# netneurolab/pypyls

Hardware: AMD Instinct MI355X
Metric: resamples/sec (perm+boot), behavioral_pls X(500x200000)/Y(500x50) fp64 (higher is better)
Workload: dtype f64

## Files before the change

pypyls_amd/csrc/plsx_k_prep.h:

```cpp
#pragma once
#include "plsx_common.h"


static __global__ void k_colmean(const double* __restrict__ X, int S, int B, double* __restrict__ mean)
{
    int b = blockIdx.x * blockDim.x + threadIdx.x;
    if (b >= B) return;
    double s = 0.0;
    for (int i = 0; i < S; ++i) s += X[(size_t)i * B + b];
    mean[b] = s / (double)S;
}

static __global__ void k_center_pad(const double* __restrict__ X, const double* __restrict__ mean,
                             int S, int B, double* __restrict__ Xc, int ldx)
{
    int b = blockIdx.x * blockDim.x + threadIdx.x;
    int i = blockIdx.y;
    if (b >= B || i >= S) return;
    Xc[(size_t)i * ldx + b] = X[(size_t)i * B + b] - mean[b];
}

static __global__ void k_cell_scale(const double* __restrict__ Xc, int ldx, int B, int J,
                             const int* __restrict__ cell_start, const int* __restrict__ cell_len,
                             double* __restrict__ Xn)
// ... 32 lines not shown
    const int* row_local = nullptr;
    const int* slice_cell0 = nullptr;
};

static __global__ void k_build_A_behav(const double* __restrict__ Y0, long long y_stride, int T, int S,
                                const int* __restrict__ cell_start, const int* __restrict__ cell_len,
                                const int* __restrict__ xsrc, const int* __restrict__ ysrc,
                                GroupLayout lay, int covariance, int scaled,
                                double* __restrict__ Afrag, size_t group_stride,
                                double* __restrict__ mom_n, int nmom_pad, int dense_ld = 0,
                                double* __restrict__ Amom = nullptr, size_t mom_stride = 0,
                                const int* __restrict__ rank = nullptr, int mom_pairs = PLSX_MOM_PAIRS,
                                int chain_cap = 0, int mom_row0 = -1, int row0 = 0)
{
    extern __shared__ double sm_b[];
    const int r = blockIdx.x, j = blockIdx.y;
    const int g = r / lay.n, rr = r % lay.n;
    const double* Y = Y0 + (size_t)r * y_stride;
    const int start = cell_start[j], len = cell_len[j];
    const int* xs = xsrc ? xsrc + (size_t)r * S : nullptr;
    const int* ys = ysrc ? ysrc + (size_t)r * S : nullptr;
    double* mean = sm_b;
    double* rstd = sm_b + T;
    __shared__ int s_cnt;
    const int tid = threadIdx.x;

    if (tid == 0) {
        int c = 0;
        for (int p = start; p < start + len; ++p) c += (xs ? xs[p] : p) >= 0;
        s_cnt = c;
    }
    __syncthreads();
    const int cnt = s_cnt;
    for (int t = tid; t < T; t += blockDim.x) {
        double s = 0.0;
        for (int p = start; p < start + len; ++p) {
            int xi = xs ? xs[p] : p;
            if (xi < 0) continue;
            int yi = ys ? ys[p] : p;
            s += Y[(size_t)yi * T + t];
        }
        double m = s / (double)cnt;
        double q = 0.0;
        for (int p = start; p < start + len; ++p) {
            int xi = xs ? xs[p] : p;
            if (xi < 0) continue;
            int yi = ys ? ys[p] : p;
            double d = Y[(size_t)yi * T + t] - m;
            q += d * d;
        }
        mean[t] = m;
        rstd[t] = covariance ? 1.0 : 1.0 / sqrt(q / (double)(cnt - 1));
    }
    __syncthreads();
    double* A = Afrag + (size_t)g * group_stride;
    const double inv_nm1 = 1.0 / (double)(cnt - 1);
    const int total = len * T;
    const bool sliced = lay.gps > 0 && !dense_ld;
    int* nxt = reinterpret_cast<int*>(sm_b + 2 * T);
    int* nfirst = nxt + len;
    const bool unique = !xs || chain_cap < 0;
    const bool chains = !unique && 2 * len <= chain_cap;
    if (chains) {
        for (int pl = tid; pl < len; pl += blockDim.x) nfirst[pl] = 0;
        __syncthreads();
        for (int pl = tid; pl < len; pl += blockDim.x) {
            const int xi = xs[start + pl];
            int nx = -1;
            if (xi >= 0)
                for (int q = pl + 1; q < len; ++q)
                    if (xs[start + q] == xi) { nx = q; break; }
            nxt[pl] = nx;
            if (nx >= 0) nfirst[nx] = 1;
        }
        __syncthreads();
    }
    for (int idx = tid; idx < total; idx += blockDim.x) {
        int pl = idx / T, t = idx - pl * T;
        int p = start + pl;
        int xi = xs ? xs[p] : p;
        if (xi < 0) continue;
        double v;
        if (chains) {
            if (nfirst[pl]) continue;
            v = 0.0;
            for (int q = pl; q >= 0; q = nxt[q]) {
                const int yq = ys ? ys[start + q] : start + q;
                v += (Y[(size_t)yq * T + t] - mean[t]) * rstd[t] * inv_nm1;
            }
        } else {
            int yi = ys ? ys[p] : p;
            v = (Y[(size_t)yi * T + t] - mean[t]) * rstd[t] * inv_nm1;
        }
        int row = rr * lay.Tp + row0 + j * T + t;
        double* dst;
        if (dense_ld) dst = Afrag + ((size_t)r * lay.Tp + j * T + t) * dense_ld + xi;
        else if (sliced) {
            const int grow = j * T + t;
            dst = Afrag + ((size_t)r * lay.gps + lay.row_slice[grow]) * group_stride +
                  afrag_off(lay.row_local[grow], xi, lay.MT);
        } else dst = A + afrag_off(row, rank ? rank[(size_t)r * S + xi] : xi, lay.MT);
        if (chains || unique) *dst = v;
        else atomicAdd(dst, v);
    }
    auto put_weight = [&](double* d0, double* d1, int pl) {
        if (chains) {
            if (nfirst[pl]) return;
            double c = 0.0;
            for (int q = pl; q >= 0; q = nxt[q]) c += 1.0;
            *d0 = c; *d1 = c;
        } else if (unique) { *d0 = 1.0; *d1 = 1.0; }
        else { atomicAdd(d0, 1.0); atomicAdd(d1, 1.0); }
    };
    if (scaled && sliced) {
        const int sa = lay.row_slice[j * T], sb = lay.row_slice[j * T + T - 1];
        for (int sl = sa; sl <= sb; ++sl) {
            const size_t gg = (size_t)r * lay.gps + sl;
            double* As = Afrag + gg * group_stride;
            const int mrow = j - lay.slice_cell0[sl];
            for (int pl = tid; pl < len; pl += blockDim.x) {
                int p = start + pl;
                int xi = xs ? xs[p] : p;
                if (xi < 0) continue;
                put_weight(As + afrag_off(lay.w0 * 16 + mrow, xi, lay.MT), As + afrag_off(lay.sq0 * 16 + mrow, xi, lay.MT), pl);
            }
            if (tid == 0) mom_n[gg * nmom_pad + mrow] = (double)cnt;
        }
    } else if (scaled && Amom) {
        const int pair = r * lay.J + j;
        double* Am = Amom + (size_t)(pair / mom_pairs) * mom_stride;
        const int mrow = pair % mom_pairs, mmt = mom_row0 >= 0 ? mom_pairs / 16 : mom_pairs / 8;
        for (int pl = tid; pl < len; pl += blockDim.x) {
            int p = start + pl;
            int xi = xs ? xs[p] : p;
            if (xi < 0) continue;
            if (mom_row0 >= 0)
                put_weight(A + afrag_off(mom_row0 + j, rank[(size_t)r * S + xi], lay.MT), Am + afrag_off(mrow, xi, mmt), pl);
            else
                put_weight(Am + afrag_off(mrow, xi, mmt), Am + afrag_off(mom_pairs + mrow, xi, mmt), pl);
        }
        if (tid == 0) mom_n[pair] = (double)cnt;
    } else if (scaled) {
        for (int pl = tid; pl < len; pl += blockDim.x) {
            int p = start + pl;
            int xi = xs ? xs[p] : p;
            if (xi < 0) continue;
            int mrow = rr * lay.J + j;
            put_weight(A + afrag_off(lay.w0 * 16 + mrow, xi, lay.MT), A + afrag_off(lay.sq0 * 16 + mrow, xi, lay.MT), pl);
        }
        if (tid == 0) mom_n[(size_t)g * nmom_pad + rr * lay.J + j] = (double)cnt;
    }
}

static __global__ __launch_bounds__(256)
void k_build_A_proj(const double* __restrict__ Y0, long long y_stride, int T, int S,
                    const int* __restrict__ cell_start, const int* __restrict__ cell_len,
                    const int* __restrict__ ysrc, const double* __restrict__ V0, int L,
                    int n, int Tp, int MT, double* __restrict__ Afrag, size_t group_stride)
{
    extern __shared__ double sm_b[];
    const int r = blockIdx.x, j = blockIdx.y;
    const int g = r / n, rr = r % n;
    const double* Y = Y0 + (size_t)r * y_stride;
    const int start = cell_start[j], len = cell_len[j];
    const int* ys = ysrc ? ysrc + (size_t)r * S : nullptr;
    double* mean = sm_b;
    double* rstd = sm_b + T;
    const int tid = threadIdx.x;
    for (int t = tid; t < T; t += blockDim.x) {
        double s = 0.0;
        for (int p = start; p < start + len; ++p) s += Y[(size_t)(ys ? ys[p] : p) * T + t];
        const double m = s / (double)len;
        double q = 0.0;
        for (int p = start; p < start + len; ++p) {
            const double d = Y[(size_t)(ys ? ys[p] : p) * T + t] - m;
            q += d * d;
        }
        mean[t] = m;
        rstd[t] = 1.0 / sqrt(q / (double)(len - 1));
    }
    __syncthreads();
    double* A = Afrag + (size_t)g * group_stride;
    const double inv_nm1 = 1.0 / (double)(len - 1);
    const double* Vj = V0 + (size_t)j * T * L;
    const int total = len * L;
    for (int idx = tid; idx < total; idx += blockDim.x) {
        const int pl = idx / L, l = idx - pl * L;
        const int p = start + pl;
        const double* y = Y + (size_t)(ys ? ys[p] : p) * T;
        double v = 0.0;
        for (int t = 0; t < T; ++t)
            v = __builtin_fma((y[t] - mean[t]) * rstd[t] * inv_nm1, Vj[(size_t)t * L + l], v);
        A[afrag_off(rr * Tp + l, p, MT)] = v;
    }
}

static __global__ void k_build_A_mc(int S, int J, int n_cond, int mean_centering,
                             const int* __restrict__ cell_of_pos,
                             const int* __restrict__ xsrc, GroupLayout lay,
                             double* __restrict__ Afrag, size_t group_stride, int dense_ld = 0, int chain_cap = 0)
{
    extern __shared__ int sm_mc[];
    __shared__ int cnt[PLSX_MAX_CELLS];
    const int r = blockIdx.x;
    const int g = r / lay.n, rr = r % lay.n;
    const int* xs = xsrc ? xsrc + (size_t)r * S : nullptr;
    const int tid = threadIdx.x;
    for (int j = tid; j < J; j += blockDim.x) cnt[j] = 0;
    __syncthreads();
    for (int p = tid; p < S; p += blockDim.x)
        if ((xs ? xs[p] : p) >= 0) atomicAdd(&cnt[cell_of_pos[p]], 1);
    __syncthreads();
    const int n_groups = J / n_cond;
    int ntot = 0;
    for (int j = 0; j < J; ++j) ntot += cnt[j];
    double* A = Afrag + (size_t)g * group_stride;
    int* nxt = sm_mc;
    int* nfirst = sm_mc + S;
    const bool unique = !xs || chain_cap < 0;
    const bool chains = !unique && 2 * S <= chain_cap;
    if (chains) {
        for (int p = tid; p < S; p += blockDim.x) nfirst[p] = 0;
        __syncthreads();
        for (int p = tid; p < S; p += blockDim.x) {
            const int xi = xs[p];
            int nx = -1;
            if (xi >= 0)
                for (int q = p + 1; q < S; ++q)
                    if (xs[q] == xi) { nx = q; break; }
            nxt[p] = nx;
            if (nx >= 0) nfirst[nx] = 1;
        }
        __syncthreads();
    }
    auto coef_of = [&](int p, int j2) -> double {
        const int j = cell_of_pos[p];
        const int gj = j / n_cond, cj = j % n_cond;
        const double own = 1.0 / (double)cnt[j];
        double coef = (j2 == j) ? own : 0.0;
        if (mean_centering == 0) {
            if (j2 / n_cond == gj) {
                int ngrp = 0;
                for (int c = 0; c < n_cond; ++c) ngrp += cnt[gj * n_cond + c];
                coef -= 1.0 / (double)ngrp;
            }
        } else if (mean_centering == 1) {
            if (j2 % n_cond == cj) coef -= own / (double)n_groups;
        } else {
            coef -= 1.0 / (double)ntot;
        }
        return coef;
    };
    for (int p = tid; p < S; p += blockDim.x) {
        int xi = xs ? xs[p] : p;
        if (xi < 0) continue;
        if (chains && nfirst[p]) continue;
        for (int j2 = 0; j2 < J; ++j2) {
            double coef;
            if (chains) {
                coef = 0.0;
                for (int q = p; q >= 0; q = nxt[q]) coef += coef_of(q, j2);
            } else coef = coef_of(p, j2);
            if (coef == 0.0) continue;
            double* dst = dense_ld ? Afrag + ((size_t)r * lay.Tp + j2) * dense_ld + xi
                                   : A + afrag_off(rr * lay.Tp + j2, xi, lay.MT);
            if (chains || unique) *dst = coef;
            else atomicAdd(dst, coef);
        }
    }
}

__device__ __forceinline__ size_t mfrag_index(int t, int l, int nks_t, int LT)
{
    const int chunk = (l >> 4) / PLSX_LT_CHUNK, lt = (l >> 4) - chunk * PLSX_LT_CHUNK;
    const int ltc = min(PLSX_LT_CHUNK, LT - chunk * PLSX_LT_CHUNK);
    return (size_t)chunk * PLSX_LT_CHUNK * nks_t * 64 + ((size_t)(t >> 2) * ltc + lt) * 64 + (t & 3) * 16 + (l & 15);
}

static __global__ __launch_bounds__(256)
void k_build_W(const double* __restrict__ Adense, int ld, int S, int Tp, int L,
               const double* __restrict__ Mfrag, int nks_t, int LT, int npg_w, int MT,
               double* __restrict__ Afrag, size_t group_stride)
{
    extern __shared__ __attribute__((aligned(16))) double sM[];
    const int r = blockIdx.x, tid = threadIdx.x;
    const double* M = Mfrag + (size_t)r * nks_t * LT * 64;
    for (int idx = tid; idx < Tp * L; idx += blockDim.x) {
        const int t = idx / L, l = idx - t * L;
        sM[idx] = M[mfrag_index(t, l, nks_t, LT)];
    }
    __syncthreads();
    const double* A = Adense + (size_t)r * Tp * ld;
    double* out = Afrag + (size_t)(r / npg_w) * group_stride;
    const int row0 = (r % npg_w) * L;
    for (int i = tid; i < S; i += blockDim.x)
        for (int l0 = 0; l0 < L; l0 += 8) {
            double w[8] = {0, 0, 0, 0, 0, 0, 0, 0};
            for (int t = 0; t < Tp; ++t) {
                const double a = A[(size_t)t * ld + i];
#pragma unroll
                for (int u = 0; u < 8; ++u) w[u] += a * sM[t * L + min(l0 + u, L - 1)];
            }
#pragma unroll
            for (int u = 0; u < 8; ++u)
                if (l0 + u < L) out[afrag_off(row0 + l0 + u, i, MT)] = w[u];
        }
}

static __global__ __launch_bounds__(256)
void k_build_Vd(const double* __restrict__ Adense, int ld, int S, int Tp, int L,
                const double* __restrict__ Mfrag, int nks_t, int LT, double* __restrict__ Vd)
{
    extern __shared__ __attribute__((aligned(16))) double sM[];
    const int r = blockIdx.x, tid = threadIdx.x;
    const double* M = Mfrag + (size_t)r * nks_t * LT * 64;
    for (int idx = tid; idx < Tp * L; idx += blockDim.x) {
        const int t = idx / L, l = idx - t * L;
        sM[idx] = M[mfrag_index(t, l, nks_t, LT)];
    }
    __syncthreads();
    const double* A = Adense + (size_t)r * Tp * ld;
    double* out = Vd + (size_t)r * L * S;
    for (int i = tid; i < S; i += blockDim.x)
        for (int l0 = 0; l0 < L; l0 += 8) {
            double w[8] = {0, 0, 0, 0, 0, 0, 0, 0};
            for (int t = 0; t < Tp; ++t) {
                const double a = A[(size_t)t * ld + i];
#pragma unroll
                for (int u = 0; u < 8; ++u) w[u] += a * sM[t * L + min(l0 + u, L - 1)];
            }
#pragma unroll
            for (int u = 0; u < 8; ++u)
                if (l0 + u < L) out[(size_t)(l0 + u) * S + i] = w[u];
        }
}

static __global__ void k_cell_moments(const double* __restrict__ Xc, int ldx, int B, int J,
                               const int* __restrict__ cell_start, const int* __restrict__ cell_len,
                               double* __restrict__ S1, double* __restrict__ S2)
{
    const int b = blockIdx.x * blockDim.x + threadIdx.x;
    if (b >= B) return;
    for (int j = 0; j < J; ++j) {
        const int r0 = cell_start[j], n = cell_len[j];
        double s = 0.0, q = 0.0;
        for (int i = r0; i < r0 + n; ++i) { const double x = Xc[(size_t)i * ldx + b]; s += x; q += x * x; }
// ... 149 lines not shown
```

pypyls_amd/csrc/plsx_k_xprod.h:

```cpp
#pragma once
#include <type_traits>
#include <utility>

template <class F, int... I>
__device__ __forceinline__ void xprod_static_for(F&& f, std::integer_sequence<int, I...>)
{
    (f(std::integral_constant<int, I>()), ...);
}
#include "plsx_common.h"
#include "plsx_k_prep.h"

#define PLSX_RSRC_FLAGS 0x00020000
template <int NT, int PASSES, bool EVEN, int STAGE>
__device__ __forceinline__ void stage_copy_buf(const double* src, double* dst, int tid, int wave)
{
    __amdgpu_buffer_rsrc_t rs = __builtin_amdgcn_make_buffer_rsrc((void*)src, (short)0, 0x7fffffff,
                                                                   PLSX_RSRC_FLAGS);
    const int voff = tid * 16;
#pragma unroll
    for (int p = 0; p < PASSES; ++p) {
        if (EVEN || p * NT + wave * 64 < STAGE / 2) {
            __builtin_amdgcn_raw_ptr_buffer_load_lds(
                rs, (__attribute__((address_space(3))) void*)(dst + (size_t)(p * NT + wave * 64) * 2),
                16, voff, p * NT * 16, 0, 0);
        }
    }
}

__device__ __forceinline__ double load_x_buf(const double* rowbase, int voff)
{
    __amdgpu_buffer_rsrc_t rs = __builtin_amdgcn_make_buffer_rsrc((void*)rowbase, (short)0, 0x7fffffff,
                                                                   PLSX_RSRC_FLAGS);
    return __builtin_bit_cast(double, __builtin_amdgcn_raw_buffer_load_b64(rs, voff, 0, 0));
}

template <int CTRL>
__device__ __forceinline__ double dpp_row_f64(double v)
{
    const int vl = __double2loint(v), vh = __double2hiint(v);
    const int lo = __builtin_amdgcn_update_dpp(vl, vl, CTRL, 0xf, 0xf, false);
    const int hi = __builtin_amdgcn_update_dpp(vh, vh, CTRL, 0xf, 0xf, false);
    return __hiloint2double(hi, lo);
}

#define PLSX_ACC_PITCH 80
template <int MT, int NW, int KT, int NSQ, int EPI = 0>
__global__ __launch_bounds__(NW * 64, 2)
void k_xprod(const double* __restrict__ Afrag, size_t group_stride,
             const double* __restrict__ X, int ldx, int nks,
             double* __restrict__ R, int ldr, int rows_per_group,
             const int* __restrict__ out_row, const int* __restrict__ mom_idx,
             const double* __restrict__ mom_n, int nmom_pad,
             int n_groups, int ncolblk, double* __restrict__ mom_out, SplitEpi se, int ntab)
{
    extern __shared__ __attribute__((aligned(16))) double smem[];
    constexpr int NT = NW * 64;
    constexpr int STAGE = KT * MT * 64;
    constexpr int STAGE_LDS = ((STAGE + 127) / 128) * 128;
    constexpr int PASSES = (STAGE + NT * 2 - 1) / (NT * 2);
    constexpr bool EVEN = (STAGE % (NT * 2)) == 0;
    const int tid = threadIdx.x;
    const int lane = tid & 63, wave = tid >> 6;
    const int sweep = blockIdx.x / (8 * ncolblk);
    const int within = blockIdx.x - sweep * (8 * ncolblk);
    int grp = sweep * 8 + (within & 7);
    int colblk = within >> 3;
    if (sweep * 8 + 8 > n_groups) {
        const int rem = n_groups - sweep * 8;
        const int cnt = (rem * ncolblk + 7) >> 3;
        const int id = (within & 7) * cnt + colblk;
        if (colblk >= cnt || id >= rem * ncolblk) return;
        grp = sweep * 8 + id / ncolblk;
        colblk = id - (id / ncolblk) * ncolblk;
    }
    const int col = colblk * (NW * 16) + wave * 16 + (lane & 15);
    const int kq = lane >> 4;

    static_assert(EPI != 7 || KT == 1 || KT == 2 || KT == 4, "EPI 7: the four k-steps of a tile row are whole stages");
    const int qblk = (EPI == 7) ? grp / max(se.J, 1) : 0;
    const int ks0 = (EPI == 7) ? qblk * (MT * 4) : 0;
    if (EPI == 7) { X += (size_t)ks0 * 4 * ldx; nks -= ks0; }
    const double* Ag = Afrag + (size_t)grp * group_stride + (size_t)ks0 * (MT * 64);
    const int swave = __builtin_amdgcn_readfirstlane(wave);
    const int xvoff = (kq * ldx + min(col, ldx - 1)) * 8;

    d4 acc[MT];
#pragma unroll
    for (int m = 0; m < MT; ++m) acc[m] = (d4){0.0, 0.0, 0.0, 0.0};

    const int nkt = nks / KT;
    constexpr bool SPLIT = (EPI == 1);
    if constexpr (SPLIT) {
        if (se.off_pre > 0 && NW == 4) {
            double* sRf = smem + se.off_pre;
            double* sRc = sRf + se.Tpp * (NW * 16);
            __amdgpu_buffer_rsrc_t rsF = __builtin_amdgcn_make_buffer_rsrc(
                (void*)(se.Rfull + (size_t)colblk * (NW * 16)), (short)0, 0x7fffffff, PLSX_RSRC_FLAGS);
            const int vo = ((lane >> 5) * ldr + (lane & 31) * 2) * 8;
            for (int j = swave; j < se.Tpp / 2; j += NW)
                __builtin_amdgcn_raw_ptr_buffer_load_lds(
                    rsF, (__attribute__((address_space(3))) void*)(sRf + j * 128), 16, vo, j * 2 * ldr * 8, 0, 0);
            __amdgpu_buffer_rsrc_t rsC = __builtin_amdgcn_make_buffer_rsrc(
                (void*)(se.rowc + (size_t)grp * MT * 16 * 5), (short)0, 0x7fffffff, PLSX_RSRC_FLAGS);
            for (int pc = swave; pc < (MT * 16 * 5 + 127) / 128; pc += NW)
                __builtin_amdgcn_raw_ptr_buffer_load_lds(
                    rsC, (__attribute__((address_space(3))) void*)(sRc + pc * 128), 16, lane * 16, pc * 1024, 0, 0);
        }
    }
    stage_copy_buf<NT, PASSES, EVEN, STAGE>(Ag, smem, tid, swave);
    double xb[KT];
#pragma unroll
    for (int s = 0; s < KT; ++s)
        xb[s] = load_x_buf(X + (size_t)(s * 4) * ldx, xvoff);
#pragma unroll
    for (int s = 0; s < KT; ++s) asm volatile("" : "+v"(xb[s]));
    __syncthreads();

    auto pass = [&](int kt, auto na) {
        constexpr int NA = decltype(na)::value;
        const int cur = kt & 1;
        const int kn = min(kt + 1, nkt - 1);
        double xn[KT];
        stage_copy_buf<NT, PASSES, EVEN, STAGE>(Ag + (size_t)kn * STAGE, smem + (cur ^ 1) * STAGE_LDS, tid, swave);
#pragma unroll
        for (int s = 0; s < KT; ++s)
            xn[s] = load_x_buf(X + (size_t)((kn * KT + s) * 4) * ldx, xvoff);
        const double* sA = smem + cur * STAGE_LDS + lane;
#pragma unroll
        for (int s = 0; s < KT; ++s) {
            const double b = xb[s];
            const double bsq = (NSQ > 0) ? b * b : 0.0;
#pragma unroll
            for (int m = 0; m < NA; ++m)
                acc[m] = mfma_f64(sA[(s * MT + m) * 64], (m < MT - NSQ) ? b : bsq, acc[m]);
        }
#pragma unroll
        for (int s = 0; s < KT; ++s) xb[s] = xn[s];
        __syncthreads();
    };
    int kt_first = 0;
    if constexpr (EPI == 7) {
        xprod_static_for([&](auto mm) {
#pragma unroll
            for (int j = 0; j < 4 / KT; ++j) {
                const int kt = (4 / KT) * decltype(mm)::value + j;
                if (kt < nkt) pass(kt, std::integral_constant<int, decltype(mm)::value + 1>());
            }
        }, std::make_integer_sequence<int, MT>());
        kt_first = min(nkt, 4 * MT / KT);
    }
    for (int kt = kt_first; kt < nkt; ++kt) pass(kt, std::integral_constant<int, MT>());

    constexpr int W0 = (EPI == 9) ? 0 : MT - 2 * NSQ, SQ0 = MT - NSQ, NMOM = NSQ * 16;
    if constexpr (EPI == 10) {
        static_assert(NSQ == 0 && NW == 4, "EPI 10 is the fixed-X block");
        double* sP = smem;
#pragma unroll
        for (int m = 0; m < MT; ++m)
#pragma unroll
            for (int i = 0; i < 4; ++i) {
                double q = acc[m][i] * acc[m][i];
                q += dpp_row_f64<0x128>(q);
                q += dpp_row_f64<0x124>(q);
                q += dpp_row_f64<0x4e>(q);
                q += dpp_row_f64<0xb1>(q);
                if ((lane & 15) == 0) sP[wave * (MT * 16) + m * 16 + kq + 4 * i] = q;
            }
        __syncthreads();
        const int rows = se.accB;
        double* pp = se.acc_sum + ((size_t)colblk * n_groups + grp) * rows;
        for (int row = tid; row < rows; row += NT)
            pp[row] = ((sP[row] + sP[MT * 16 + row]) + sP[2 * MT * 16 + row]) + sP[3 * MT * 16 + row];
        return;
    }
    if constexpr (EPI == 9) {
        static_assert(MT == NSQ, "EPI 9 runs every tile against X^2");
#pragma unroll
        for (int j = 0; j < MT; ++j)
#pragma unroll
            for (int i = 0; i < 4; ++i) {
                const int pair = grp * (MT * 16) + j * 16 + kq + 4 * i;
                if (pair >= se.npairs || col >= ldr) continue;
                se.scale[(size_t)pair * ldr + col] = acc[j][i];
            }
        return;
    }
    if constexpr (EPI == 6) {
        static_assert(MT == 2 * NSQ, "EPI 6 is a moment-only instantiation");
#pragma unroll
        for (int j = 0; j < NSQ; ++j)
#pragma unroll
            for (int i = 0; i < 4; ++i) {
                const int pair = grp * (NSQ * 16) + j * 16 + kq + 4 * i;
                if (pair >= se.npairs || col >= ldr) continue;
                se.scale[(size_t)pair * ldr + col] = acc[j][i];
                se.scale2[(size_t)pair * ldr + col] = acc[NSQ + j][i];
            }
        return;
    }
    if constexpr (EPI == 4) {
        static_assert(MT == 2 * NSQ, "EPI 4 is the moment-only instantiation");
#pragma unroll
        for (int j = 0; j < NSQ; ++j)
#pragma unroll
            for (int i = 0; i < 4; ++i) {
                const int pair = grp * (NSQ * 16) + j * 16 + kq + 4 * i;
                if (pair >= se.npairs || col >= ldr) continue;
                const double m1 = acc[j][i], m2 = acc[NSQ + j][i];
                const double nn = mom_n[pair];
                const double var = (m2 - m1 * m1 / nn) / (nn - 1.0);
                se.scale[(size_t)pair * ldr + col] = (var > 0.0) ? sd_rsqrt(var) : 0.0;
            }
        return;
    }
    if constexpr (EPI == 3) {
        const int nmu = se.npairs;
        double* sS3 = smem;
        int* s_out = reinterpret_cast<int*>(smem + (size_t)nmu * (NW * 16));
        int* s_mom = s_out + MT * 16;
        const double* sc0 = se.scale + (size_t)grp * nmu * ldr + colblk * (NW * 16);
        for (int idx = tid; idx < nmu * (NW * 16); idx += NT) {
            const int mi = idx / (NW * 16), c = idx - mi * (NW * 16);
            sS3[idx] = sc0[(size_t)mi * ldr + c];
        }
        for (int i = tid; i < MT * 16; i += NT) { s_out[i] = out_row[i]; s_mom[i] = mom_idx[i]; }
        __syncthreads();
        double* Rg = R + (size_t)grp * rows_per_group * ldr + col;
        const int cw = wave * 16 + (lane & 15);
        const int rows_valid = min(rows_per_group, se.accB - grp * rows_per_group);
#pragma unroll
        for (int m = 0; m < MT; ++m) {
            int orow[4];
            double sc[4];
#pragma unroll
            for (int i = 0; i < 4; ++i) {
                const int row = m * 16 + kq + 4 * i;
                orow[i] = s_out[row];
                const int mi = s_mom[row];
                sc[i] = mi >= 0 ? sS3[mi * (NW * 16) + cw] : 1.0;
            }
#pragma unroll
            for (int i = 0; i < 4; ++i)
                if (orow[i] >= 0 && orow[i] < rows_valid) Rg[(size_t)orow[i] * ldr] = acc[m][i] * sc[i];
        }
        return;
    }
    if constexpr (EPI == 7) {
        if (NW > 4 && col >= ldr) return;
        const int s0 = qblk * (MT * 16);
        const int Srows = se.accB;
        const double* Xc = X + col - (size_t)(ks0 * 4) * ldx;
        double part = 0.0;
#pragma unroll
        for (int m = 0; m < MT; ++m) {
            double xv[4];
#pragma unroll
            for (int i = 0; i < 4; ++i) {
                const int sr = s0 + m * 16 + kq + 4 * i;
                const double x = Xc[(size_t)min(sr, Srows - 1) * ldx];
                xv[i] = sr < Srows ? x : 0.0;
            }
#pragma unroll
            for (int i = 0; i < 4; ++i) part = __builtin_fma(xv[i], acc[m][i], part);
            asm volatile("" : "+v"(part));
        }
        part += __shfl_xor(part, 16);
        part += __shfl_xor(part, 32);
        if (kq == 0) se.acc_sum[(size_t)grp * ldr + col] = part;
        return;
    }
    if constexpr (EPI == 2) {
        constexpr int ACCP = NW * 16 + 16;
        constexpr int BCW = NW * 16;
        const int L = se.accL;
        double* sU = smem;
        double* sV = smem + (size_t)L * ACCP;
        double* sT = sV + (size_t)L * ACCP;
        int* s_l = reinterpret_cast<int*>(sT + 32 * ACCP);
        for (int i = tid; i < 2 * L * ACCP; i += NT) smem[i] = 0.0;
        for (int i = tid; i < MT * 16; i += NT) s_l[i] = out_row[i];
        const int cw = wave * 16 + (lane & 15);
#pragma unroll
        for (int m0 = 0; m0 < MT; m0 += 2) {
            __syncthreads();
#pragma unroll
            for (int mm = 0; mm < 2; ++mm)
#pragma unroll
                for (int i = 0; i < 4; ++i)
                    if (m0 + mm < MT) sT[(mm * 16 + kq + 4 * i) * ACCP + cw] = acc[m0 + mm][i];
            __syncthreads();
            for (int idx = tid; idx < L * BCW; idx += NT) {
                const int l = idx / BCW, c = idx - l * BCW;
                double u = sU[l * ACCP + c], v2 = sV[l * ACCP + c];
                for (int rl = 0; rl < 32 && m0 * 16 + rl < MT * 16; ++rl)
                    if (s_l[m0 * 16 + rl] == l) { const double v = sT[rl * ACCP + c]; u += v; v2 += v * v; }
                sU[l * ACCP + c] = u; sV[l * ACCP + c] = v2;
            }
        }
        __syncthreads();
        const int b0 = colblk * (NW * 16);
        double* ps = se.acc_sum + (size_t)grp * se.accB * L;
        double* pq = se.acc_sq + (size_t)grp * se.accB * L;
        for (int idx = tid; idx < NW * 16 * L; idx += NT) {
            const int c = idx / L, l = idx - c * L;
            if (b0 + c < se.accB) {
                ps[(size_t)(b0 + c) * L + l] = sU[l * ACCP + c];
                pq[(size_t)(b0 + c) * L + l] = sV[l * ACCP + c];
            }
        }
        return;
    }
    if constexpr (SPLIT && NSQ > 0) {
        const int nmu = se.nmu;
        const bool pre = se.off_pre > 0 && NW == 4;
        double* w5 = smem + wave * (5 * nmu * 16);
        int* s_out = reinterpret_cast<int*>(smem + NW * 5 * nmu * 16);
        int* s_mom = s_out + MT * 16;
        const double* sRf = smem + se.off_pre;
        double* s_rc = pre ? smem + se.off_pre + se.Tpp * (NW * 16)
                           : reinterpret_cast<double*>(s_mom + MT * 16);
        const int pitch2 = 2 * se.Tpp;
        for (int i = tid; i < MT * 16; i += NT) {
            const int orw = out_row[i];
            s_out[i] = orw < 0 ? -1 : (orw | ((orw % pitch2) << 20));
            s_mom[i] = mom_idx[i];
// ... 462 lines not shown
```

pypyls_amd/csrc/plsx_xprod.hip:

```cpp
#include "plsx_internal.h"

using namespace plsxi;

namespace plsxi {

template <int MT, int NW, int KT, int NSQ>
int launch_xprod_t(plsx_ctx* ctx, int groups, hipStream_t st)
{
    const size_t stage = (size_t)2 * (((size_t)KT * MT * 64 + 127) / 128) * 128 * 8;
    const size_t epi = (size_t)NW * 2 * NSQ * 16 * 16 * 8 + (size_t)2 * MT * 16 * 4;
    const size_t lds = std::max(stage, epi);
    HIPCHK(set_lds(k_xprod<MT, NW, KT, NSQ>, lds));
    const int ncolblk = ctx->Bpad / (NW * 16);
    dim3 grid(ncolblk * round_up(groups, 8)), block(NW * 64);
    KTimer tm(ctx, KC_XPROD, st);
    hipLaunchKernelGGL((k_xprod<MT, NW, KT, NSQ>), grid, block, lds, st,
                       ptr<double>(ctx->Afrag) + (size_t)ctx->afrag_group0 * ctx->group_stride, ctx->group_stride,
                       ptr<double>(ctx->Xc), ctx->Bpad,
                       ctx->nks, ptr<double>(ctx->R), ctx->Bpad, ctx->npg * ctx->Tpp,
                       ptr<int>(ctx->out_row), ptr<int>(ctx->mom_idx), ptr<double>(ctx->mom_n),
                       std::max(ctx->nmom_pad, 0), groups, ncolblk, ctx->mom_out_arg,
                       SplitEpi{nullptr, nullptr, nullptr, nullptr, nullptr, 0, 0}, std::max(ctx->gps, 1));
    LAUNCHCHK();
    return 0;
}

int launch_xprod(plsx_ctx* ctx, int groups, hipStream_t st)
{
    if (ctx->MT == 16)
        switch (ctx->MT - ctx->sq0) {
            case 0: return launch_xprod_t<16, 4, 1, 0>(ctx, groups, st);
            case 1: return launch_xprod_t<16, 4, 1, 1>(ctx, groups, st);
            case 2: return launch_xprod_t<16, 4, 1, 2>(ctx, groups, st);
            default: return launch_xprod_t<16, 4, 1, 3>(ctx, groups, st);
        }
    switch (ctx->MT - ctx->sq0) {
        case 0: return launch_xprod_t<24, 4, 1, 0>(ctx, groups, st);
        case 1: return launch_xprod_t<24, 4, 1, 1>(ctx, groups, st);
        case 2: return launch_xprod_t<24, 4, 1, 2>(ctx, groups, st);
        default: return launch_xprod_t<24, 4, 1, 3>(ctx, groups, st);
    }
}

int launch_xprod_acc(plsx_ctx* ctx, const double* Afrag, size_t gstride, int groups, int L, hipStream_t st)
{
    constexpr int MT = 24, KT = 1;
    const size_t stage = (size_t)2 * (((size_t)KT * MT * 64 + 127) / 128) * 128 * 8;
    SplitEpi se;
    memset(&se, 0, sizeof(se));
    se.acc_sum = ptr<double>(ctx->psum); se.acc_sq = ptr<double>(ctx->psq); se.accL = L; se.accB = ctx->B;
    KTimer tm(ctx, KC_XPROD, st);
    if ((2 * (size_t)L + 32) * (8 * 16 + 16) * 8 + MT * 16 * 4 <= 96 * 1024) {
        constexpr int NW = 8;
        const size_t lds = std::max(stage, ((size_t)2 * L + 32) * (NW * 16 + 16) * 8 + (size_t)MT * 16 * 4);
        HIPCHK(set_lds(k_xprod<MT, NW, KT, 0, 2>, lds));
        const int ncolblk = ceil_div(ctx->Bpad, NW * 16);
        hipLaunchKernelGGL((k_xprod<MT, NW, KT, 0, 2>), dim3(ncolblk * round_up(groups, 8)), dim3(NW * 64), lds, st,
                           Afrag, gstride, ptr<double>(ctx->Xc), ctx->Bpad, ctx->nks, (double*)nullptr, ctx->Bpad, 0,
                           ptr<int>(ctx->out_row_w), (const int*)nullptr, (const double*)nullptr, 0, groups, ncolblk,
                           (double*)nullptr, se, 1);
    } else {
        constexpr int NW = 4;
        const size_t lds = std::max(stage, ((size_t)2 * L + 32) * PLSX_ACC_PITCH * 8 + (size_t)MT * 16 * 4);
        HIPCHK(set_lds(k_xprod<MT, NW, KT, 0, 2>, lds));
        const int ncolblk = ctx->Bpad / (NW * 16);
        hipLaunchKernelGGL((k_xprod<MT, NW, KT, 0, 2>), dim3(ncolblk * round_up(groups, 8)), dim3(NW * 64), lds, st,
                           Afrag, gstride, ptr<double>(ctx->Xc), ctx->Bpad, ctx->nks, (double*)nullptr, ctx->Bpad, 0,
                           ptr<int>(ctx->out_row_w), (const int*)nullptr, (const double*)nullptr, 0, groups, ncolblk,
                           (double*)nullptr, se, 1);
    }
    LAUNCHCHK();
    return 0;
}

static int stage_ksteps(int nks) { return nks % 3 == 0 ? 3 : (nks % 2 == 0 ? 2 : 1); }

template <int MT, int NW, int KT, int EPI>
int launch_moments_t(plsx_ctx* ctx, size_t stride, int groups, SplitEpi se, hipStream_t st)
{
    constexpr int NSQ = (EPI == 9) ? MT : MT / 2;
    const size_t lds = (size_t)2 * (((size_t)KT * MT * 64 + 127) / 128) * 128 * 8;
    HIPCHK(set_lds(k_xprod<MT, NW, KT, NSQ, EPI>, lds));
    const int ncolblk = ceil_div(ctx->Bpad, NW * 16);
    hipLaunchKernelGGL((k_xprod<MT, NW, KT, NSQ, EPI>), dim3(ncolblk * round_up(groups, 8)), dim3(NW * 64), lds, st,
                       ptr<double>(ctx->Afrag_m), stride, ptr<double>(ctx->Xc), ctx->Bpad, ctx->nks,
                       (double*)nullptr, ctx->Bpad, 0, (const int*)nullptr, (const int*)nullptr,
                       ptr<double>(ctx->momn_m), 0, groups, ncolblk, (double*)nullptr, se, 1);
    LAUNCHCHK();
    return 0;
}

template <int MT, int NW, int EPI>
int launch_moments(plsx_ctx* ctx, size_t stride, int groups, SplitEpi se, hipStream_t st)
{
    if constexpr (EPI == 4 || EPI == 9) {
        const int kt = stage_ksteps(ctx->nks);
        if (kt == 3) return launch_moments_t<MT, NW, 3, EPI>(ctx, stride, groups, se, st);
        if (kt == 2) return launch_moments_t<MT, NW, 2, EPI>(ctx, stride, groups, se, st);
    }
    return launch_moments_t<MT, NW, 1, EPI>(ctx, stride, groups, se, st);
}

template <int KT>
int launch_xprod_fixed_t(plsx_ctx* ctx, int groups, hipStream_t st)
{
    constexpr int MT = 25, NW = 4;
    const size_t stage = (size_t)2 * (((size_t)KT * MT * 64 + 127) / 128) * 128 * 8;
    const size_t lds = std::max(stage, (size_t)2 * MT * 16 * 4);
    HIPCHK(set_lds(k_xprod<MT, NW, KT, 0>, lds));
    const int ncolblk = ctx->Bpad / (NW * 16);
    dim3 grid(ncolblk * round_up(groups, 8)), block(NW * 64);
    KTimer tm(ctx, KC_XPROD, st);
    hipLaunchKernelGGL((k_xprod<MT, NW, KT, 0>), grid, block, lds, st,
                       ptr<double>(ctx->Afrag), ctx->group_stride_f, ptr<double>(ctx->Xn), ctx->Bpad,
                       ctx->nks, ptr<double>(ctx->R), ctx->Bpad, ctx->npgf * ctx->Tpp,
                       ptr<int>(ctx->out_row_f), ptr<int>(ctx->mom_idx_f), ptr<double>(ctx->mom_n), 0,
                       groups, ncolblk, (double*)nullptr, SplitEpi{nullptr, nullptr, nullptr, nullptr, nullptr, 0, 0}, 1);
    LAUNCHCHK();
    return 0;
}

int run_xprod_fixed(plsx_ctx* ctx, const int* ysrc, int nres, hipStream_t st, const double* ystack)
{
    const int groups = ceil_div(nres, ctx->npgf);
    if (int e = ensure_scratch(ctx, groups)) return e;
    if (ctx->timing) ctx->timed_units += nres;
    ctx->last_compact_n = 0;
    HIPCHK(hipMemsetAsync(ctx->Afrag.p, 0, (size_t)groups * ctx->group_stride_f * 8, st));
    GroupLayout lay;
    lay.n = ctx->npgf; lay.Tp = ctx->Tp; lay.J = ctx->J; lay.T = ctx->T; lay.MT = ctx->MTf;
    lay.w0 = ctx->MTf; lay.sq0 = ctx->MTf; lay.Tpp = ctx->Tpp;
    {
        dim3 grid(nres, ctx->J), block(256);
        const size_t lds = (size_t)2 * ctx->T * 8;
        hipLaunchKernelGGL(k_build_A_behav, grid, block, lds, st, ystack ? ystack : ptr<double>(ctx->Y),
                           ystack ? (long long)ctx->S * ctx->T : 0LL, ctx->T, ctx->S,
                           ptr<int>(ctx->cell_start), ptr<int>(ctx->cell_len), (const int*)nullptr, ysrc, lay,
                           0, 0, ptr<double>(ctx->Afrag), ctx->group_stride_f, ptr<double>(ctx->mom_n), 16);
        LAUNCHCHK();
    }
    switch (stage_ksteps(ctx->nks)) {
        case 3: return launch_xprod_fixed_t<3>(ctx, groups, st);
        case 2: return launch_xprod_fixed_t<2>(ctx, groups, st);
        default: return launch_xprod_fixed_t<1>(ctx, groups, st);
    }
}

template <int KT>
int launch_xprod_fixed_norms_t(plsx_ctx* ctx, int groups, SplitEpi se, hipStream_t st)
{
    constexpr int MT = 25, NW = 4;
    const size_t stage = (size_t)2 * (((size_t)KT * MT * 64 + 127) / 128) * 128 * 8;
    const size_t lds = std::max(stage, (size_t)NW * MT * 16 * 8);
    HIPCHK(set_lds(k_xprod<MT, NW, KT, 0, 10>, lds));
    const int ncolblk = ctx->Bpad / (NW * 16);
    dim3 grid(ncolblk * round_up(groups, 8)), block(NW * 64);
    KTimer tm(ctx, KC_XPROD, st);
    hipLaunchKernelGGL((k_xprod<MT, NW, KT, 0, 10>), grid, block, lds, st,
                       ptr<double>(ctx->Afrag), ctx->group_stride_f, ptr<double>(ctx->Xn), ctx->Bpad,
                       ctx->nks, (double*)nullptr, ctx->Bpad, ctx->npgf * ctx->Tpp,
                       (const int*)nullptr, (const int*)nullptr, (const double*)nullptr, 0,
                       groups, ncolblk, (double*)nullptr, se, 1);
    LAUNCHCHK();
    return 0;
}

int run_xprod_fixed_norms(plsx_ctx* ctx, const int* ysrc, int nres, hipStream_t st, const double* ystack, double* out_sv)
{
    const int groups = ceil_div(nres, ctx->npgf), rows = ctx->npgf * ctx->Tp;
    const int ncolblk = ctx->Bpad / 64;
    if (int e = ensure(ctx, ctx->Afrag, (size_t)groups * ctx->group_stride_f * 8 + 4096)) return e;
    if (int e = ensure(ctx, ctx->ppart, (size_t)ncolblk * groups * rows * 8)) return e;
    if (ctx->timing) ctx->timed_units += nres;
    ctx->last_compact_n = 0;
    HIPCHK(hipMemsetAsync(ctx->Afrag.p, 0, (size_t)groups * ctx->group_stride_f * 8, st));
    {
        KTimer tm(ctx, KC_BUILD, st);
        hipLaunchKernelGGL(k_build_A_proj, dim3(nres, ctx->J), dim3(256), (size_t)2 * ctx->T * 8, st,
                           ystack ? ystack : ptr<double>(ctx->Y), ystack ? (long long)ctx->S * ctx->T : 0LL, ctx->T, ctx->S,
                           ptr<int>(ctx->cell_start), ptr<int>(ctx->cell_len), ysrc, ptr<double>(ctx->V0), ctx->L,
                           ctx->npgf, ctx->Tp, ctx->MTf, ptr<double>(ctx->Afrag), ctx->group_stride_f);
        LAUNCHCHK();
    }
    SplitEpi se;
    memset(&se, 0, sizeof(se));
    se.acc_sum = ptr<double>(ctx->ppart); se.accB = rows;
    int e;
    switch (stage_ksteps(ctx->nks)) {
        case 3: e = launch_xprod_fixed_norms_t<3>(ctx, groups, se, st); break;
        case 2: e = launch_xprod_fixed_norms_t<2>(ctx, groups, se, st); break;
        default: e = launch_xprod_fixed_norms_t<1>(ctx, groups, se, st); break;
    }
    if (e) return e;
    KTimer tm(ctx, KC_SMALL, st);
    const long long count = (long long)nres * ctx->Tp;
    hipLaunchKernelGGL(k_rownorm_finish, dim3((unsigned)((count + 255) / 256)), dim3(256), 0, st, ptr<double>(ctx->ppart),
                       ncolblk, groups, rows, ctx->npgf, ctx->Tp, nres, out_sv);
    LAUNCHCHK();
    return 0;
}

template <int MT>
int launch_xprod_data(plsx_ctx* ctx, int groups, SplitEpi se, hipStream_t st)
{
    constexpr int NW = 4, KT = 1;
    const size_t stage = (size_t)2 * (((size_t)KT * MT * 64 + 127) / 128) * 128 * 8;
    const size_t epi = (size_t)se.npairs * NW * 16 * 8 + (size_t)2 * MT * 16 * 4;
    const size_t lds = std::max(stage, epi);
    HIPCHK(set_lds(k_xprod<MT, NW, KT, 0, 3>, lds));
    const int ncolblk = ctx->Bpad / (NW * 16);
    KTimer tm(ctx, KC_XPROD, st);
    hipLaunchKernelGGL((k_xprod<MT, NW, KT, 0, 3>), dim3(ncolblk * round_up(groups, 8)), dim3(NW * 64), lds, st,
                       ptr<double>(ctx->Afrag), ctx->group_stride_d, ptr<double>(ctx->Xc), ctx->Bpad, ctx->nks,
                       ptr<double>(ctx->R), ctx->Bpad, ctx->npg_d * ctx->Tpp, ptr<int>(ctx->out_row_d),
                       ptr<int>(ctx->mom_idx_d), (const double*)nullptr, 0, groups, ncolblk, (double*)nullptr, se, 1);
    LAUNCHCHK();
    return 0;
}

int run_xprod_sepmom(plsx_ctx* ctx, const int* xsrc, const int* ysrc, int nres, hipStream_t st,
                     const double* ystack, long long ystride)
{
    const int npairs = nres * ctx->J;
    const int groups_d = ceil_div(nres, ctx->npg_d), groups_m = ceil_div(npairs, PLSX_MOM_PAIRS);
    const size_t mstride = (size_t)ctx->nks * 24 * 64;
    if (int e = ensure(ctx, ctx->Afrag_m, (size_t)groups_m * mstride * 8 + 4096)) return e;
    if (int e = ensure(ctx, ctx->momn_m, (size_t)round_up(npairs, PLSX_MOM_PAIRS) * 8)) return e;
    if (int e = ensure(ctx, ctx->scale, (size_t)round_up(std::max(npairs, groups_d * ctx->npg_d * ctx->J), 8) * ctx->Bpad * 8))
        return e;
    HIPCHK(hipMemsetAsync(ctx->Afrag.p, 0, (size_t)groups_d * ctx->group_stride_d * 8, st));
    HIPCHK(hipMemsetAsync(ctx->Afrag_m.p, 0, (size_t)groups_m * mstride * 8, st));
    GroupLayout lay;
    lay.n = ctx->npg_d; lay.Tp = ctx->Tp; lay.J = ctx->J; lay.T = ctx->T; lay.MT = ctx->MTd;
    lay.w0 = ctx->MTd; lay.sq0 = ctx->MTd; lay.Tpp = ctx->Tpp;
    {
        KTimer tm(ctx, KC_BUILD, st);
        int cap = 0;
        const size_t blds = build_lds_behav(ctx, &cap);
        hipLaunchKernelGGL(k_build_A_behav, dim3(nres, ctx->J), dim3(256), blds, st,
                           ystack ? ystack : ptr<double>(ctx->Y), ystack ? ystride : 0LL, ctx->T, ctx->S,
                           ptr<int>(ctx->cell_start), ptr<int>(ctx->cell_len), xsrc, ysrc, lay, ctx->cov, 1,
                           ptr<double>(ctx->Afrag), ctx->group_stride_d, ptr<double>(ctx->momn_m), 0, 0,
                           ptr<double>(ctx->Afrag_m), mstride, (const int*)nullptr, PLSX_MOM_PAIRS, cap);
        LAUNCHCHK();
    }
    SplitEpi se;
    memset(&se, 0, sizeof(se));
    se.scale = ptr<double>(ctx->scale);
    {
        se.npairs = npairs;
        KTimer tm(ctx, KC_MOM, st);
        if (int e = launch_moments<24, 8, 4>(ctx, mstride, groups_m, se, st)) return e;
    }
    se.npairs = ctx->npg_d * ctx->J;
    se.accB = nres * ctx->Tpp;
    switch (ctx->MTd) {
        case 24: return launch_xprod_data<24>(ctx, groups_d, se, st);
        case 22: return launch_xprod_data<22>(ctx, groups_d, se, st);
        default: return launch_xprod_data<16>(ctx, groups_d, se, st);
    }
}

MomLayout moment_layout(const plsx_ctx* ctx, int npairs)
{
    const int t192 = ceil_div(npairs, 192) * 24, t128 = ceil_div(npairs, 128) * 16;
    MomLayout m;
    m.pairs = (t128 * 6 < t192 * 5) ? 128 : 192;
    m.mt = m.pairs / 8;
    m.groups = ceil_div(npairs, m.pairs);
    m.stride = (size_t)ctx->nks * m.mt * 64;
    return m;
}

MomLayout moment2_layout(const plsx_ctx* ctx, int npairs)
{
    const int t384 = ceil_div(npairs, 384) * 24, t256 = ceil_div(npairs, 256) * 16;
    MomLayout m;
    m.pairs = (t256 * 6 < t384 * 5) ? 256 : 384;
    m.mt = m.pairs / 16;
    m.groups = ceil_div(npairs, m.pairs);
    m.stride = (size_t)ctx->nks * m.mt * 64;
    return m;
}

template <int EPI>
int launch_moment_blocks(plsx_ctx* ctx, const MomLayout& ml, SplitEpi se, hipStream_t st)
{
    constexpr int NW = (EPI == 6) ? 4 : 8;
    KTimer tm(ctx, KC_MOM, st);
    if (ml.mt == 24) return launch_moments<24, NW, EPI>(ctx, ml.stride, ml.groups, se, st);
    return launch_moments<16, NW, EPI>(ctx, ml.stride, ml.groups, se, st);
}

int ensure_compact_maps(plsx_ctx* ctx)
{
    if (ctx->has_compact_maps) return 0;
    const int rows = ceil_div(ctx->Tp, 16) * 16;
    std::vector<int> orow(rows, -1), mrow(rows, -1);
    for (int t = 0; t < ctx->Tp; ++t) { orow[t] = t; mrow[t] = t / ctx->T; }
    if (int e = ensure(ctx, ctx->out_row_c, rows * sizeof(int))) return e;
    if (int e = ensure(ctx, ctx->mom_idx_c, rows * sizeof(int))) return e;
    HIPCHK(hipMemcpy(ctx->out_row_c.p, orow.data(), rows * sizeof(int), hipMemcpyHostToDevice));
    HIPCHK(hipMemcpy(ctx->mom_idx_c.p, mrow.data(), rows * sizeof(int), hipMemcpyHostToDevice));
    ctx->has_compact_maps = 1;
    return 0;
}

int launch_moment_blocks_raw(plsx_ctx* ctx, const MomLayout& ml, SplitEpi se, hipStream_t st)
{
    return launch_moment_blocks<6>(ctx, ml, se, st);
}

bool compact_boot_ok(const plsx_ctx* ctx)
{
    if (!(ctx->scaled && ctx->method == PLSX_BEHAVIORAL && ctx->gps == 0 && ctx->Tp <= 208 && !ctx->mom_out_arg &&
          ctx->J <= 32 && ctx->S <= 8192 && (long long)ctx->Kpad * ctx->Bpad * 8 < (1LL << 31)))
        return false;
    const int force = ctx->opt[OPT_COMPACT_BOOT_ALWAYS] ? 1 : (ctx->opt[OPT_NO_COMPACT_BOOT] ? -1 : 0);
    if (force) return force > 0;
    const int mt = ceil_div(ctx->Tp, 16);
    const double rows = (mt >= 2 && ctx->Tp - (mt - 1) * 16 <= 4) ? (mt - 1) * 16 + 4 : mt * 16;
    const double cost_c = 0.66 * 1.25 * rows / 16.0;
    const int npg_dense = ctx->sepmom ? ctx->npg_d : ctx->npg, mt_dense = ctx->sepmom ? ctx->MTd : ctx->MT;
    return cost_c * 1.1 < (double)mt_dense / npg_dense && npg_dense <= 16;
}

int compact_boot_ksteps(int mt) { return mt == 4 ? PLSX_CKT : std::max(1, 12 / mt); }

bool compact_moment_rows(const plsx_ctx* ctx)
{
    if (ctx->opt[OPT_NO_MOMENT_ROWS]) return false;
// ... 240 lines not shown
```

Before: 6367.

## Tile projection build through LDS and simplify fixed-norm xprod epilogue

k_build_A_proj now stages the standardized Y rows for a chunk of subjects in LDS, optionally caches the V projection matrix in LDS, and computes four subjects per thread so each V load is reused. This replaces per-element global reads of Y and V. In the fixed-X norm xprod kernel the MFMA operands are swapped, explicit sched_group_barrier interleaving of loads and MFMAs is added, and the DPP cross-lane square reduction is replaced by per-lane FMA sums written to a larger LDS buffer that is reduced afterwards. The cost is more LDS per block, which may reduce occupancy.

```diff
diff --git a/pypyls_amd/csrc/plsx_k_prep.h b/pypyls_amd/csrc/plsx_k_prep.h
--- a/pypyls_amd/csrc/plsx_k_prep.h
+++ b/pypyls_amd/csrc/plsx_k_prep.h
@@ -208,6 +208,19 @@
     }
 }
 
+#define PLSX_PROJ_LDS_DOUBLES 6144
+__host__ __device__ constexpr bool build_A_proj_vlds(int T, int L) { return T * L <= PLSX_PROJ_LDS_DOUBLES / 2; }
+__host__ __device__ constexpr int build_A_proj_chunk(int T, int L)
+{
+    const int room = (PLSX_PROJ_LDS_DOUBLES - 2 * T - (build_A_proj_vlds(T, L) ? T * L : 0)) / T;
+    return room >= 64 ? 64 : room < 4 ? 4 : room & ~3;
+}
+__host__ __device__ constexpr size_t build_A_proj_lds(int T, int L)
+{
+    return ((size_t)2 * T + (size_t)build_A_proj_chunk(T, L) * T + (build_A_proj_vlds(T, L) ? (size_t)T * L : 0)) * 8;
+}
+
+template <bool VLDS>
 static __global__ __launch_bounds__(256)
 void k_build_A_proj(const double* __restrict__ Y0, long long y_stride, int T, int S,
                     const int* __restrict__ cell_start, const int* __restrict__ cell_len,
@@ -220,9 +233,15 @@
     const double* Y = Y0 + (size_t)r * y_stride;
     const int start = cell_start[j], len = cell_len[j];
     const int* ys = ysrc ? ysrc + (size_t)r * S : nullptr;
+    const int ch = build_A_proj_chunk(T, L);
     double* mean = sm_b;
     double* rstd = sm_b + T;
+    double* sZ = sm_b + 2 * T;
+    double* sV = sZ + ch * T;
+    const double* Vj = V0 + (size_t)j * T * L;
     const int tid = threadIdx.x;
+    if (VLDS)
+        for (int i = tid; i < T * L; i += blockDim.x) sV[i] = Vj[i];
     for (int t = tid; t < T; t += blockDim.x) {
         double s = 0.0;
         for (int p = start; p < start + len; ++p) s += Y[(size_t)(ys ? ys[p] : p) * T + t];
@@ -238,16 +257,31 @@
     __syncthreads();
     double* A = Afrag + (size_t)g * group_stride;
     const double inv_nm1 = 1.0 / (double)(len - 1);
-    const double* Vj = V0 + (size_t)j * T * L;
-    const int total = len * L;
-    for (int idx = tid; idx < total; idx += blockDim.x) {
-        const int pl = idx / L, l = idx - pl * L;
-        const int p = start + pl;
-        const double* y = Y + (size_t)(ys ? ys[p] : p) * T;
-        double v = 0.0;
-        for (int t = 0; t < T; ++t)
-            v = __builtin_fma((y[t] - mean[t]) * rstd[t] * inv_nm1, Vj[(size_t)t * L + l], v);
-        A[afrag_off(rr * Tp + l, p, MT)] = v;
+    const double* Vs = VLDS ? sV : Vj;
+    for (int c0 = 0; c0 < len; c0 += ch) {
+        const int nr = min(ch, len - c0);
+        for (int idx = tid; idx < nr * T; idx += blockDim.x) {
+            const int pl = idx / T, t = idx - pl * T;
+            const int p = start + c0 + pl;
+            sZ[idx] = (Y[(size_t)(ys ? ys[p] : p) * T + t] - mean[t]) * rstd[t] * inv_nm1;
+        }
+        __syncthreads();
+        const int nq = (nr + 3) >> 2;
+        for (int idx = tid; idx < nq * L; idx += blockDim.x) {
+            const int q = idx / L, l = idx - q * L;
+            const double* z = sZ + (size_t)q * 4 * T;
+            double v[4] = {0.0, 0.0, 0.0, 0.0};
+            for (int t = 0; t < T; ++t) {
+                const double w = Vs[(size_t)t * L + l];
+#pragma unroll
+                for (int i = 0; i < 4; ++i) v[i] = __builtin_fma(z[i * T + t], w, v[i]);
+            }
+            const int p0 = start + c0 + q * 4;
+#pragma unroll
+            for (int i = 0; i < 4; ++i)
+                if (q * 4 + i < nr) A[afrag_off(rr * Tp + l, p0 + i, MT)] = v[i];
+        }
+        __syncthreads();
     }
 }
 
diff --git a/pypyls_amd/csrc/plsx_k_xprod.h b/pypyls_amd/csrc/plsx_k_xprod.h
--- a/pypyls_amd/csrc/plsx_k_xprod.h
+++ b/pypyls_amd/csrc/plsx_k_xprod.h
@@ -32,15 +32,6 @@
     __amdgpu_buffer_rsrc_t rs = __builtin_amdgcn_make_buffer_rsrc((void*)rowbase, (short)0, 0x7fffffff,
                                                                    PLSX_RSRC_FLAGS);
     return __builtin_bit_cast(double, __builtin_amdgcn_raw_buffer_load_b64(rs, voff, 0, 0));
-}
-
-template <int CTRL>
-__device__ __forceinline__ double dpp_row_f64(double v)
-{
-    const int vl = __double2loint(v), vh = __double2hiint(v);
-    const int lo = __builtin_amdgcn_update_dpp(vl, vl, CTRL, 0xf, 0xf, false);
-    const int hi = __builtin_amdgcn_update_dpp(vh, vh, CTRL, 0xf, 0xf, false);
-    return __hiloint2double(hi, lo);
 }
 
 #define PLSX_ACC_PITCH 80
@@ -131,8 +122,18 @@
             const double b = xb[s];
             const double bsq = (NSQ > 0) ? b * b : 0.0;
 #pragma unroll
-            for (int m = 0; m < NA; ++m)
-                acc[m] = mfma_f64(sA[(s * MT + m) * 64], (m < MT - NSQ) ? b : bsq, acc[m]);
+            for (int m = 0; m < NA; ++m) {
+                if constexpr (EPI == 10) acc[m] = mfma_f64(b, sA[(s * MT + m) * 64], acc[m]);
+                else acc[m] = mfma_f64(sA[(s * MT + m) * 64], (m < MT - NSQ) ? b : bsq, acc[m]);
+            }
+        }
+        if constexpr (EPI == 10) {
+            __builtin_amdgcn_sched_group_barrier(0x100, 7, 0);
+#pragma unroll
+            for (int i = 0; i < (KT * MT) / 2; ++i) {
+                __builtin_amdgcn_sched_group_barrier(0x008, 2, 0);
+                __builtin_amdgcn_sched_group_barrier(0x100, 1, 0);
+            }
         }
 #pragma unroll
         for (int s = 0; s < KT; ++s) xb[s] = xn[s];
@@ -154,23 +155,29 @@
     constexpr int W0 = (EPI == 9) ? 0 : MT - 2 * NSQ, SQ0 = MT - NSQ, NMOM = NSQ * 16;
     if constexpr (EPI == 10) {
         static_assert(NSQ == 0 && NW == 4, "EPI 10 is the fixed-X block");
+        constexpr int PP = MT * 16;
         double* sP = smem;
-#pragma unroll
-        for (int m = 0; m < MT; ++m)
-#pragma unroll
-            for (int i = 0; i < 4; ++i) {
-                double q = acc[m][i] * acc[m][i];
-                q += dpp_row_f64<0x128>(q);
-                q += dpp_row_f64<0x124>(q);
-                q += dpp_row_f64<0x4e>(q);
-                q += dpp_row_f64<0xb1>(q);
-                if ((lane & 15) == 0) sP[wave * (MT * 16) + m * 16 + kq + 4 * i] = q;
-            }
+        double* sq = sP + (wave * 4 + kq) * PP + (lane & 15);
+#pragma unroll
+        for (int m = 0; m < MT; ++m) {
+            double q = acc[m][0] * acc[m][0];
+            q = __builtin_fma(acc[m][1], acc[m][1], q);
+            q = __builtin_fma(acc[m][2], acc[m][2], q);
+            q = __builtin_fma(acc[m][3], acc[m][3], q);
+            sq[m * 16] = q;
+        }
         __syncthreads();
         const int rows = se.accB;
         double* pp = se.acc_sum + ((size_t)colblk * n_groups + grp) * rows;
-        for (int row = tid; row < rows; row += NT)
-            pp[row] = ((sP[row] + sP[MT * 16 + row]) + sP[2 * MT * 16 + row]) + sP[3 * MT * 16 + row];
+        for (int row = tid; row < rows; row += NT) {
+            double w[NW];
+#pragma unroll
+            for (int v = 0; v < NW; ++v) {
+                const double* p = sP + v * 4 * PP + row;
+                w[v] = (p[0] + p[PP]) + (p[2 * PP] + p[3 * PP]);
+            }
+            pp[row] = (w[0] + w[1]) + (w[2] + w[3]);
+        }
         return;
     }
     if constexpr (EPI == 9) {
diff --git a/pypyls_amd/csrc/plsx_xprod.hip b/pypyls_amd/csrc/plsx_xprod.hip
--- a/pypyls_amd/csrc/plsx_xprod.hip
+++ b/pypyls_amd/csrc/plsx_xprod.hip
@@ -151,7 +151,7 @@
 {
     constexpr int MT = 25, NW = 4;
     const size_t stage = (size_t)2 * (((size_t)KT * MT * 64 + 127) / 128) * 128 * 8;
-    const size_t lds = std::max(stage, (size_t)NW * MT * 16 * 8);
+    const size_t lds = std::max(stage, (size_t)NW * 4 * MT * 16 * 8);
     HIPCHK(set_lds(k_xprod<MT, NW, KT, 0, 10>, lds));
     const int ncolblk = ctx->Bpad / (NW * 16);
     dim3 grid(ncolblk * round_up(groups, 8)), block(NW * 64);
@@ -176,7 +176,8 @@
     HIPCHK(hipMemsetAsync(ctx->Afrag.p, 0, (size_t)groups * ctx->group_stride_f * 8, st));
     {
         KTimer tm(ctx, KC_BUILD, st);
-        hipLaunchKernelGGL(k_build_A_proj, dim3(nres, ctx->J), dim3(256), (size_t)2 * ctx->T * 8, st,
+        auto kern = build_A_proj_vlds(ctx->T, ctx->L) ? k_build_A_proj<true> : k_build_A_proj<false>;
+        hipLaunchKernelGGL(kern, dim3(nres, ctx->J), dim3(256), build_A_proj_lds(ctx->T, ctx->L), st,
                            ystack ? ystack : ptr<double>(ctx->Y), ystack ? (long long)ctx->S * ctx->T : 0LL, ctx->T, ctx->S,
                            ptr<int>(ctx->cell_start), ptr<int>(ctx->cell_len), ysrc, ptr<double>(ctx->V0), ctx->L,
                            ctx->npgf, ctx->Tp, ctx->MTf, ptr<double>(ctx->Afrag), ctx->group_stride_f);
```

Measured after the change: 6520 (median of 6 runs). 2.4% higher.
